# bjack205/rsLQR

Hardware: AMD Instinct MI355X
Metric: LQR solves/sec (nx=12,nu=4,N=256,batch=1024 per GPU) (higher is better)
Workload: dtype f64; 1 GPU; nx=12 nu=4 N=256 batch=1024 per GPU, fp64, factor+solve per step; parallelism=batch-sharded x1, no data-path collective, ranks_seen=1, flags=0, schedule=reduced-fused2

## Files before the change

### include/ndlqr_hip.h

```cpp
#ifndef NDLQR_HIP_H_
#define NDLQR_HIP_H_

#include <stddef.h>
#include <stdint.h>

#ifdef __cplusplus
extern "C" {
#endif

typedef struct NdlqrHipCtx NdlqrHipCtx;

int ndlqr_hip_device_count(void);
const char* ndlqr_hip_last_error(void);

NdlqrHipCtx* ndlqr_hip_create(int nstates, int ninputs, int nhorizon, int batch, int device);
#define NDLQR_CREATE_NO_PAD 1u
NdlqrHipCtx* ndlqr_hip_create_ex(int nstates, int ninputs, int nhorizon, int batch, int device, unsigned create_flags);
void ndlqr_hip_destroy(NdlqrHipCtx* ctx);
int ndlqr_hip_set_flags(NdlqrHipCtx* ctx, unsigned flags);
unsigned ndlqr_hip_get_flags(const NdlqrHipCtx* ctx);
int ndlqr_hip_set_stream(NdlqrHipCtx* ctx, void* hip_stream);
void* ndlqr_hip_get_stream(NdlqrHipCtx* ctx);

int ndlqr_hip_upload_inputs(NdlqrHipCtx* ctx, int p0, int count, const double* AB,
// ... 90 lines not shown
int ndlqr_hip_download_selection(NdlqrHipCtx* ctx, int knot0, int nknots, unsigned blocks, double* out);
int ndlqr_hip_time_shard_top_doubles(NdlqrHipCtx* ctx, int G);
int ndlqr_hip_time_shard_factor(NdlqrHipCtx* ctx, int g, int G);
int ndlqr_hip_time_shard_export(NdlqrHipCtx* ctx, int G, double* buf);
int ndlqr_hip_time_shard_import(NdlqrHipCtx* ctx, int G, const double* buf);
int ndlqr_hip_time_shard_finish(NdlqrHipCtx* ctx, int g, int G);
void* ndlqr_hip_host_alloc(size_t bytes);
void ndlqr_hip_host_free(void* p);
void* ndlqr_hip_device_alloc(size_t bytes);
void ndlqr_hip_device_free(void* p);
int ndlqr_hip_copy(void* dst, const void* src, size_t bytes);

int ndlqr_hip_download_solutions(NdlqrHipCtx* ctx, int p0, int count, double* soln);
int ndlqr_hip_download_rhs_blocks(NdlqrHipCtx* ctx, int p, double* z_full);
int ndlqr_hip_download_factors(NdlqrHipCtx* ctx, int p, double* fact);
int ndlqr_hip_factors_valid(const NdlqrHipCtx* ctx);
int ndlqr_hip_pack_solutions_device(NdlqrHipCtx* ctx, double* dst);
int ndlqr_hip_kkt_residual(NdlqrHipCtx* ctx, double* res, double* bnorm);
int ndlqr_hip_cholesky_failures(NdlqrHipCtx* ctx);
int ndlqr_hip_download_failure_counts(NdlqrHipCtx* ctx, int* counts);
const char* ndlqr_hip_schedule(const NdlqrHipCtx* ctx);
int ndlqr_hip_compact_level1(const NdlqrHipCtx* ctx);
int ndlqr_hip_level1_paired(const NdlqrHipCtx* ctx);

int ndlqr_hip_profile_slots(NdlqrHipCtx* ctx);
int ndlqr_hip_profile_get(NdlqrHipCtx* ctx, int slot, char* name, int name_cap, double* total_ms,
                          int* launches);
int ndlqr_hip_profile_reset(NdlqrHipCtx* ctx);

int ndlqr_hip_gemm(int tA, int tB, int m, int n, int k, double alpha, const double* A, int lda,
                   const double* B, int ldb, double beta, double* C, int ldc);
int ndlqr_hip_potrf_lower(int n, double* A, int lda);
int ndlqr_hip_potrs_lower(int n, int nrhs, const double* L, int ldl, double* B, int ldb);
int ndlqr_hip_trsv_lower(int n, int nrhs, const double* L, int ldl, double* B, int ldb, int transposed);

#ifdef __cplusplus
}
#endif
#endif
```

### rslqr_amd/api.py

```python
import ctypes as C
import os
import re

import numpy as np

from . import build as _build

FLAG_STRICT_FP = 1
FLAG_GENERIC = 2
FLAG_PROFILE = 4
FLAG_KEEP_FACT = 8
FLAG_KEEP_RECORDS = 16
SOLN_LAMBDA, SOLN_STATE, SOLN_INPUT, SOLN_ONLY = 1, 2, 4, 8
GRAD_A, GRAD_B, GRAD_Q, GRAD_R, GRAD_q, GRAD_r, GRAD_d, GRAD_x0 = 1, 2, 4, 8, 16, 32, 64, 128
GRAD_NAMES = ("A", "B", "Q", "R", "q", "r", "d", "x0")
GRADD_A, GRADD_B, GRADD_Q, GRADD_H, GRADD_R, GRADD_q, GRADD_r, GRADD_d, GRADD_x0 = 1, 2, 4, 8, 16, 32, 64, 128, 256
GRAD_DENSE_NAMES = ("A", "B", "Q", "H", "R", "q", "r", "d", "x0")

ERR_INVALID = -1
ERR_NO_DEVICE = -2
ERR_NOT_SPD = -3

dp = C.POINTER(C.c_double)

# ... 285 lines not shown
    proto("ndlqr_BatchSetBoxAcceleration", ci, vp, ci, cd, cd)
    proto("ndlqr_CopyBatchBoxAcceleration", ci, vp, C.POINTER(ci), C.POINTER(ci), dp, C.POINTER(ci))
    proto("ndlqr_SolveBatchBoxAdjoint", ci, vp, dp, C.POINTER(NdLqrBoxSettingsFull), C.POINTER(ci), C.POINTER(ci))
    proto("ndlqr_BatchBoundGradients", ci, vp, C.c_uint, dp, dp, dp, dp)
    proto("ndlqr_PolishBatchBoxConstrained", ci, vp, C.POINTER(NdLqrPolishSettings), C.POINTER(ci), C.POINTER(ci))
    proto("ndlqr_hip_download_polish_codes", ci, vp, C.POINTER(C.c_ubyte))
    proto("ndlqr_SolveBatchPolishedAdjoint", ci, vp, dp, C.POINTER(NdLqrPolishSettings), C.POINTER(ci), C.POINTER(ci))
    proto("ndlqr_hip_factor_count", C.c_ulonglong, vp)
    proto("ndlqr_hip_set_stream", ci, vp, vp)
    proto("ndlqr_hip_get_stream", vp, vp)
    proto("ndlqr_hip_profile_slots", ci, vp)
    proto("ndlqr_hip_profile_get", ci, vp, ci, C.c_char_p, ci, dp, C.POINTER(ci))
    proto("ndlqr_hip_profile_reset", ci, vp)
    proto("ndlqr_hip_device_pointers", ci, vp, C.POINTER(vp))
    proto("ndlqr_hip_staged_io", ci, vp, C.POINTER(dp), C.POINTER(dp), C.POINTER(dp), C.POINTER(dp))
    proto("ndlqr_hip_download_rhs_blocks", ci, vp, ci, dp)
    proto("ndlqr_hip_upload_inputs", ci, vp, ci, ci, dp, dp, dp)
    proto("ndlqr_hip_factors_valid", ci, vp)
    proto("ndlqr_hip_schedule", C.c_char_p, vp)
    if hasattr(L, "ndlqr_hip_compact_level1"):
        proto("ndlqr_hip_compact_level1", C.c_int, vp)
    if hasattr(L, "ndlqr_hip_level1_paired"):
        proto("ndlqr_hip_level1_paired", C.c_int, vp)
    proto("ndlqr_hip_set_pipeline_depth", ci, vp, ci)
    proto("ndlqr_hip_pipeline_depth", ci, vp)
    proto("ndlqr_hip_pack_solutions_device", ci, vp, vp)
    proto("ndlqr_hip_gemm", ci, ci, ci, ci, ci, ci, cd, dp, ci, dp, ci, cd, dp, ci)
    proto("ndlqr_hip_potrf_lower", ci, ci, dp, ci)
    proto("ndlqr_hip_potrs_lower", ci, ci, ci, dp, ci, dp, ci)
    proto("ndlqr_hip_trsv_lower", ci, ci, ci, dp, ci, dp, ci, ci)
    _LIB = L
    return L


def pinned_empty(shape):
    import weakref
    count = int(np.prod(shape))
    L = lib()
    ptr = L.ndlqr_HostAlloc(max(count, 1) * 8)
    if not ptr:
        raise MemoryError("ndlqr_HostAlloc(%d bytes) failed" % (count * 8))
    buf = (C.c_double * max(count, 1)).from_address(ptr)
    arr = np.ctypeslib.as_array(buf)[:count].reshape(shape)
    weakref.finalize(buf, L.ndlqr_HostFree, C.c_void_p(ptr))
    return arr

# ... 788 lines not shown
        err = self.L.ndlqr_CopyBatchCholeskyFailureCounts(self.h, out.ctypes.data_as(C.POINTER(C.c_int)))
        if err:
            raise RuntimeError("ndlqr_CopyBatchCholeskyFailureCounts failed: %d" % err)
        return out

    def profile(self):
        out = {}
        for slot in range(self.L.ndlqr_hip_profile_slots(self.ctx)):
            name = C.create_string_buffer(64)
            ms, cnt = C.c_double(0), C.c_int(0)
            self.L.ndlqr_hip_profile_get(self.ctx, slot, name, 64, C.byref(ms), C.byref(cnt))
            out[name.value.decode()] = (ms.value, cnt.value)
        return out

    def schedule(self):
        return self.L.ndlqr_hip_schedule(self.ctx).decode()

    def compact_level1(self):
        return hasattr(self.L, "ndlqr_hip_compact_level1") and bool(self.L.ndlqr_hip_compact_level1(self.ctx))

    def level1_paired(self):
        return hasattr(self.L, "ndlqr_hip_level1_paired") and bool(self.L.ndlqr_hip_level1_paired(self.ctx))

    def set_pipeline_depth(self, depth):
        return self.L.ndlqr_hip_set_pipeline_depth(self.ctx, depth)

    def pipeline_depth(self):
        return self.L.ndlqr_hip_pipeline_depth(self.ctx)

    def profile_reset(self):
        self.L.ndlqr_hip_profile_reset(self.ctx)
```

### rslqr_amd/csrc/hip_context.hpp

```cpp
#pragma once
#include <hip/hip_runtime.h>

#include <cstdio>
#include <cstdlib>
#include <cstring>
#include <initializer_list>
#include <string>
#include <utility>
#include <vector>

#include "ndlqr.h"
#include "ndlqr_hip.h"

#include "kernels_common.hpp"

#pragma GCC visibility push(hidden)
int ndlqr_hip_fail(const char* what, hipError_t e);
struct NdlqrHipCtx;
int ndlqr_hip_ensure_F(NdlqrHipCtx* c);
#pragma GCC visibility pop
#define HIP_TRY(expr)                                                  \
  do {                                                                 \
    hipError_t e_ = (expr);                                            \
    if (e_ != hipSuccess) return ndlqr_hip_fail(#expr, e_);            \
// ... 6 lines not shown
  if (lds <= kLdsDefaultDynamic) return hipSuccess;
  return hipFuncSetAttribute(reinterpret_cast<const void*>(kernel), hipFuncAttributeMaxDynamicSharedMemorySize, (int)lds);
}


enum { SLOT_LEAF = 0, SLOT_SEP, SLOT_SCHUR, SLOT_BOUNDARY, SLOT_APPLY, SLOT_BOTTOM, SLOT_UPPER, SLOT_TOP, SLOT_COUNT };

struct PendingEvent {
  int slot;
  hipEvent_t start, stop;
};

enum class Family { None, Small, GenericReduced, GenericKnot };

struct KeptState {
  Family family = Family::None;
  bool time_shard = false;
  bool rec_complete = false;
  bool rec_compact = false;
  bool fact_valid = false;
  const char* schedule = "none";
  bool rec1_compact = false;
  bool level1_paired = false;
  void forget_factorisation() { rec_complete = fact_valid = false; }
};

struct CapturedChain {
  hipGraphExec_t exec = nullptr;
  unsigned flags = 0;
  hipStream_t stream = nullptr;
  unsigned apply = 0;
  void reset() {
    if (exec) (void)hipGraphExecDestroy(exec);
    exec = nullptr;
  }
};

struct KnotSlice {
  int knot0 = 0, nknots = 0;
  unsigned blocks = 7u;
  bool valid(int N, unsigned allowed) const {
    return knot0 >= 0 && nknots > 0 && knot0 + nknots <= N && (blocks & 7u) && !(blocks & ~allowed);
  }
  size_t width(const ndlqr::Dims& u) const {
    return ((blocks & 1u) ? u.n : 0) + ((blocks & 2u) ? u.n : 0) + ((blocks & 4u) ? u.m : 0);
  }
// ... 58 lines not shown
  DevBuf<double> red;
  DevBuf<double> ytop;
  DevBuf<double> z;
  DevBuf<double> rhs;
  DevBuf<double> xfer;
  DevBuf<int> tree_cnt;
  PinnedBuf<int> h_fail;
  hipStream_t stream = nullptr;
  hipEvent_t ev_start = nullptr, ev_stop = nullptr;
  unsigned long long rhs_gen[4] = {};
  CapturedChain graph;
  bool ready = false;
  hipError_t ensure_xfer(const ndlqr::Dims& u) { return xfer.ensure((size_t)u.batch * u.N * u.rows + (size_t)u.batch * u.n); }
};


struct DevKnobs {
  int rowbcast = -1;
  int tree = -1;
  int backsub_cols = -1;
  int fuse2 = -1;
  int compact1 = -1;
  int pair1 = -1;
  int pipeline = 2;
  bool no_top = false;
  int top_levels = 3;
  bool no_mfma = false;
  int sep_threads = 0;
  int mult_threads = 0;
  bool no_reduced_generic = false;
  bool no_pad = false;
  bool alt_priority_set = false;
  int alt_priority = 0;
};

struct AdjointState {
  DevBuf<double> rhs, z;
  DevBuf<double> save;
  unsigned long long gen = 0;
  unsigned long long rhs_stamp = 0;
  hipError_t ensure_save(const ndlqr::Dims& d) { return save.ensure(2 * (size_t)d.batch * d.N * d.n); }
  hipError_t ensure(const ndlqr::Dims& d, hipStream_t st) {
    return first_error({rhs.ensure(doubles_z(d)), z.ensure_zeroed(doubles_z(d), st), ensure_save(d)});
  }
};

// ... 308 lines not shown
```

### rslqr_amd/csrc/kernels_bottom_reduced.hpp

```cpp
#pragma once
#include "kernels_dpp.hpp"
#include "kernels_small.hpp"

namespace ndlqr {

typedef double acc4_t __attribute__((ext_vector_type(4)));

template <int NX>
struct McPitch {
  static constexpr int SP = 18, WP = 17;
};

template <int NX, class Hook>
__device__ __forceinline__ void factor_tail_mc(const int lane, const acc4_t& c, const double (&ra)[(NX + 3) / 4],
                                               const double (&rb)[(NX + 3) / 4], const double* Wm, acc4_t& X0,
                                               acc4_t& X1, Hook hook) {
  constexpr int KS = (NX + 3) / 4, WP = McPitch<NX>::WP;
  int lane_o = lane;
  asm volatile("" : "+v"(lane_o));
  const int li = lane_o & 15, lk = lane_o >> 4;
  double wt[KS], wa[KS], b0[KS];
#pragma unroll
  for (int q = 0; q < KS; ++q) {
    wt[q] = Wm[(4 * q + lk) * WP + li];
// ... 439 lines not shown
template <int NX>
__device__ __forceinline__ double* lstore_of(const int store_l, double* F, double* rec, const Dims& d, const int b,
                                             const int level, const int s) {
  return store_l == 2 ? rb_lrec<NX>(rec, d, b, s) : (store_l ? Fblk(F, d, b, level, s + 1) : nullptr);
}

template <int NX, int NU, bool BOTTOM = true>
struct alignas(16) ReducedLds {
  static constexpr int W = NX + NU, ROWS = 2 * NX + NU, WP = (W % 2 == 0) ? W + 2 : W;
  static constexpr int SLOT = RedSlot<NX>::SIZE, NSC = McWyLayout<NX>::SIZE;
  static constexpr int NB0 = BOTTOM ? 4 * NX * WP : 0, NB1 = SLOT + NX * WP;
  static constexpr int NB2 = BOTTOM ? McPairLayout<NX>::SIZE : 0;
  static constexpr int NB3 = BOTTOM ? McPairYLayout<NX>::SIZE : 0;
  static constexpr int NB01 = (NB0 > NB1 ? NB0 : NB1) > NSC ? (NB0 > NB1 ? NB0 : NB1) : NSC;
  static constexpr int NB23 = NB2 > NB3 ? NB2 : NB3;
  static constexpr int NBUF = NB01 > NB23 ? NB01 : NB23;
  static constexpr int NRQ = BOTTOM ? 4 * W : (W + NX + 1) / 2 * 2, NRH = BOTTOM ? 4 * ROWS : (NX + W + 2 * NX + 1) / 2 * 2;
  double buf[NBUF];
  double rq[NRQ];
  double rh[NRH];
#ifdef NDLQR_DEV_LDS_PAD
  double dev_pad[BOTTOM ? NDLQR_DEV_LDS_PAD / 8 : 1];
#endif
};

template <int NX, int NU, bool TREE, class LdsT, bool EXT = false>
__device__ __forceinline__ void reduced_separator_mc(const Dims& d, const int l, const int base, const int b,
                                                     const int lane, const double* __restrict__ AB,
                                                     const double* __restrict__ QR,
                                                     const double* __restrict__ rhs, double* red,
                                                     double* __restrict__ rec, double* F, int* __restrict__ info,
                                                     const int store_l, LdsT& lds, const double* slot_ext = nullptr) {
  constexpr int W = NX + NU, NN = NX * NX, KSN = (NX + 3) / 4;
  constexpr int WP = ReducedLds<NX, NU>::WP, SLOT = RedSlot<NX>::SIZE;
  const double* slot = EXT ? slot_ext : lds.buf;
  double* abs_ = lds.buf + SLOT;
  double* rq = lds.rq;
  double* zs = lds.rh;
  static_assert(LdsT::NRQ >= W + NX && LdsT::NRH >= NX + W + 2 * NX, "the shared arrays are large enough for a level");
  const int N = d.N;
  const int T = 2 << l, s = base + (1 << l) - 1;
  const bool hasA = base > 0, hasB = base + T < N;
  const int li = lane & 15, lk = lane >> 4;
  const int ri = li < NX ? li : NX - 1;
  SEG_INIT();
  const bool leftchild = (base & T) == 0;
// ... 173 lines not shown
  using PY = McPairYLayout<NX>;
  constexpr int KSN = (NX + 3) / 4;
  int lane = lane_in;
  asm volatile("" : "+v"(lane));
  const int li = lane & 15, lk = lane >> 4;
  const bool hasA = k0 > 0, hasB = k0 + 4 < d.N, leftchild = (k0 & 4) == 0;
  RedSlot<NX> sa = red_slot<NX>(red, d, b, hasA ? k0 - 1 : 3);
  RedSlot<NX> sb = red_slot<NX>(red, d, b, hasB ? k0 + 3 : 3);
  if (slotA) sa.p = slotA;
  if (slotB) sb.p = slotB;
  double y0[KSN], y1[KSN];
  acc4_t Z0 = {0.0, 0.0, 0.0, 0.0}, Z1 = {0.0, 0.0, 0.0, 0.0};
#pragma unroll
  for (int q = 0; q < KSN; ++q) {
    y0[q] = buf[PY::tile(0, 0) + (4 * q + lk) * PY::YP + li];
    y1[q] = buf[PY::tile(0, 1) + (4 * q + lk) * PY::YP + li];
    Z0[q] = y0[q]; Z1[q] = y1[q];
  }
  acc4_t g00, g01, g11, unused;
  gram_mc<NX, true, true, false, true>(y0, y1, Z0, Z1, g00, g01, unused, g11);
  push_mc<NX>(lane, hasA, hasB, leftchild, sa, sb, g00, g01, g11, hd.park_a, hd.cb_t, hd.park_b11, StorePlain(), StorePlain());
}

template <int NX, int NU, bool TREE, bool REDIRECT, bool C1 = false, bool P1 = false>
__device__ __forceinline__ void bottom_group_mc(const Dims& d, const int k0, const int b, const int lane,
                                                const double* __restrict__ AB, const double* __restrict__ QR,
                                                const double* __restrict__ rhs, double* red, double* __restrict__ rec,
                                                double* F, int* __restrict__ info, const int store_l, const int compact0,
                                                ReducedLds<NX, NU>& lds, double* slotA, double* slotB,
                                                const bool with_m = false, acc4_t* c_m = nullptr,
                                                Pair1Hand* hand = nullptr);
template <int NX, int NU, bool C1 = false, bool P1 = false>
__global__ __launch_bounds__(128) __attribute__((amdgpu_waves_per_eu(4))) void bottom8_reduced_mc(
    Dims d, const double* __restrict__ AB, const double* __restrict__ QR, const double* __restrict__ rhs, double* red,
    double* __restrict__ rec, int* __restrict__ info) {
  __shared__ ReducedLds<NX, NU> lds[2];
  __shared__ __attribute__((aligned(16))) double mslot[RedSlot<NX>::SIZE];
  const int wave = __builtin_amdgcn_readfirstlane(threadIdx.x >> 6), b = blockIdx.y;
  const int kw = (blockIdx.x + d.xoff) * 8;
  int lane = threadIdx.x & 63;
  for (int e = threadIdx.x; e < RedSlot<NX>::SIZE; e += 128) mslot[e] = 0.0;
  __syncthreads();
  acc4_t c_m = {0.0, 0.0, 0.0, 0.0};
  if constexpr (P1) {
    static_assert(C1, "the paired pass is the Y-only pass of compact level-1 records");
    static_assert(McPair1Layout<NX>::SIZE <= ReducedLds<NX, NU>::NBUF, "tile and couplings of t fit the wavefront's buffer");
    Pair1Hand hd;
    bottom_group_mc<NX, NU, false, true, true, true>(d, kw + 4 * wave, b, lane, AB, QR, rhs, red, rec, nullptr, info, 0, 1,
                                                     lds[wave], nullptr, nullptr, wave == 0, &c_m, &hd);
    pair1_exchange_mc<NX>(lane, hd.c_t, hd.ca_t, hd.cb_t, lds[wave].buf);
    __syncthreads();
    if (wave == 0) {
      double* rec_t0 = rec + ((size_t)b * d.N + kw + 1) * (2 * NX * NX + NX);
      if (chol_pair1_y_mc<NX>(lane, lds[0].buf, lds[1].buf, rec_t0, rec_t0 + 4 * (2 * NX * NX + NX)) &&
          (lane == 0 || lane == 32))
        flag_failure(info, d, b);
    }
    __syncthreads();
    pair1_tail_mc<NX, NU>(d, kw + 4 * wave, b, lane, red, lds[wave].buf, hd, wave == 1 ? mslot : nullptr,
                          wave == 0 ? mslot : nullptr);
  } else {
  bottom_group_mc<NX, NU, false, true, C1>(d, kw + 4 * wave, b, lane, AB, QR, rhs, red, rec, nullptr, info, 0, 1, lds[wave],
                                       wave == 1 ? mslot : nullptr, wave == 0 ? mslot : nullptr, wave == 0, &c_m);
  }
  asm volatile("s_waitcnt vmcnt(0)" ::: "memory");
  __syncthreads();
  asm volatile("" : "+v"(lane));
  if (wave == 0) reduced_eliminate_pass_mc<NX, NU>(d, kw, b, lane, c_m, mslot, info, lds[0].buf);
  __syncthreads();
  reduced_eliminate_tail_mc<NX, NU>(d, kw, b, lane, wave == 0, red, rec, lds[0].buf);
}

template <int NX>
__device__ __forceinline__ void backsub_top_body(const Dims& d, const int b, const int t,
                                                 const double* __restrict__ recs, double* __restrict__ ytop,
                                                 double* ytop_lds, const int bp = -1, const double* zsep = nullptr);
template <int NX, int NU>
__global__ __launch_bounds__(256) __attribute__((amdgpu_waves_per_eu(4))) void reduced_top_mc(Dims d, const int l0, const double* __restrict__ AB,
                                                      const double* __restrict__ QR, const double* __restrict__ rhs,
                                                      double* red, double* __restrict__ rec, double* F,
                                                      int* __restrict__ info, const int store_l,
                                                      double* __restrict__ ytop) {
  __shared__ ReducedLds<NX, NU, false> lds[4];
  const int wave = __builtin_amdgcn_readfirstlane(threadIdx.x >> 6), b = blockIdx.x;
  for (int l = l0, s0 = 0; l < d.K;) {
    int lane = threadIdx.x & 63;
    asm volatile("" : "+v"(lane));
    const int cnt = d.N >> (l + 1);
    if (wave + s0 < cnt)
      reduced_separator_mc<NX, NU, true>(d, l, (wave + s0) * (2 << l), b, lane, AB, QR, rhs, red, rec, F, info, store_l,
                                         lds[wave]);
    s0 += 4;
    if (s0 < cnt) continue;
    s0 = 0;
    ++l;
    asm volatile("s_waitcnt vmcnt(0)" ::: "memory");
    __syncthreads();
  }
  if (ytop) backsub_top_body<NX>(d, b, threadIdx.x, rec, ytop, reinterpret_cast<double*>(&lds[0]), -1, nullptr);
}

template <int NX, int NU, bool TREE, bool REDIRECT, bool C1, bool P1>
__device__ __forceinline__ void bottom_group_mc(const Dims& d, const int k0, const int b, const int lane,
                                                const double* __restrict__ AB, const double* __restrict__ QR,
                                                const double* __restrict__ rhs, double* red, double* __restrict__ rec,
                                                double* F, int* __restrict__ info, const int store_l, const int compact0,
                                                ReducedLds<NX, NU>& lds, double* slotA, double* slotB,
                                                const bool with_m, acc4_t* c_m, Pair1Hand* hand) {
  static_assert(!P1 || (C1 && REDIRECT && !TREE), "the paired level-1 pass: the fused bottom launch with compact level-1 records");
  constexpr int W = NX + NU, ROWS = 2 * NX + NU, NN = NX * NX, KSN = (NX + 3) / 4;
  constexpr int REC = 2 * NN + NX;
  constexpr int WP = ReducedLds<NX, NU>::WP;
  double* abs_ = lds.buf;
  double* rq = lds.rq;
  double* rh = lds.rh;
  const int N = d.N;
  const int li = lane & 15, lk = lane >> 4;
  const int ri = li < NX ? li : NX - 1;
  const bool hasA = k0 > 0, hasB = k0 + 4 < N;
  SEG_INIT();

  {
    const double* abm = AB + ((size_t)b * N + k0) * NX * W;
    const double* q0 = QR + ((size_t)b * N + k0) * W;
    const double* r0 = rhs + ((size_t)b * N + k0) * ROWS;
    constexpr int NQ = 4 * W, IQ = (NQ + 63) / 64, NR = 4 * ROWS, IR = (NR + 63) / 64;
    double qv[IQ], rv[IR];
#pragma unroll
    for (int it = 0; it < IQ; ++it) { const int e = lane + 64 * it; qv[it] = q0[e < NQ ? e : NQ - 1]; }
#pragma unroll
    for (int it = 0; it < IR; ++it) { const int e = lane + 64 * it; rv[it] = r0[e < NR ? e : NR - 1]; }
    if constexpr (W % 2 == 0) {
      constexpr int NA = 4 * NX * W / 2, IA = (NA + 63) / 64;
      double2 t[IA];
#pragma unroll
      for (int it = 0; it < IA; ++it) {
        const int e = lane + 64 * it;
        t[it] = reinterpret_cast<const double2*>(abm)[e < NA ? e : NA - 1];
      }
#pragma unroll
      for (int it = 0; it < IA; ++it) {
        const int e = lane + 64 * it, ec = e < NA ? e : NA - 1, row = ec / (W / 2), c2 = ec - row * (W / 2);
        reinterpret_cast<double2*>(&abs_[row * WP])[c2] = t[it];
      }
    } else {
      constexpr int NA = 4 * NX * W, IA = (NA + 63) / 64;
      double t[IA];
#pragma unroll
      for (int it = 0; it < IA; ++it) { const int e = lane + 64 * it; t[it] = abm[e < NA ? e : NA - 1]; }
#pragma unroll
      for (int it = 0; it < IA; ++it) { const int e = lane + 64 * it; abs_[e < NA ? e : NA - 1] = t[it]; }
    }
#pragma unroll
    for (int it = 0; it < IQ; ++it) {
      const int e = lane + 64 * it, ec = e < NQ ? e : NQ - 1, kn = ec / W, c = ec - kn * W;
      rq[ec] = 1.0 / qv[it];
      if (e < NQ && !positive_finite(qv[it]) && !(k0 + kn == N - 1 && c >= NX)) flag_failure(info, d, b);
    }
#pragma unroll
    for (int it = 0; it < IR; ++it) { const int e = lane + 64 * it; rh[e < NR ? e : NR - 1] = rv[it]; }
  }
  wave_lds_sync();
  SEG(20);

  auto none = [](int) { return 0.0; };
  acc4_t c_s0;
// ... 90 lines not shown
  }
  wave_lds_sync();
  SEG(21);

  using Pair = McPairLayout<NX>;
  if (chol_pair_mc<NX>(lane, c_s0, c_s2, lds.buf, store_l ? Fblk(F, d, b, 0, k0 + 1) : nullptr,
                       store_l ? Fblk(F, d, b, 0, k0 + 3) : nullptr) &&
      (lane == 0 || lane == 32))
    flag_failure(info, d, b);
  SEG(30);
  factor_tail_mc<NX>(lane, c_s0, ra0, rb0, lds.buf + Pair::W_A, X0, X1, hook_s0);
  store_record_mc<NX>(myrec, lane, hasA, true, X0, X1);
  factor_tail_mc<NX>(lane, c_s2, ra2, rb2, lds.buf + Pair::W_B, X0, X1, hook_s2);
  store_record_mc<NX>(myrec + 2 * REC, lane, true, hasB, X0, X1);
  SEG(35);
  }
  if constexpr (P1) {
    hand->c_t = c_t; hand->ca_t = ca_t; hand->cb_t = cb_t; hand->park_a = park_a; hand->park_b11 = park_b11;
    return;
  }
  double wcol[NX];
  {
    constexpr int TP = 17;
    static_assert(2 * 16 * TP <= ReducedLds<NX, NU>::NBUF, "both coupling tiles fit the buffer");
    double* ta = lds.buf;
    double* tb = lds.buf + 16 * TP;
    wave_lds_sync();
#pragma unroll
    for (int g = 0; g < 4; ++g) {
      ta[(lk + 4 * g) * TP + li] = -ca_t[g];
      tb[(lk + 4 * g) * TP + li] = -cb_t[g];
    }
    wave_lds_sync();
    const int h = lane & 31;
    const bool is_a = h < NX, is_b = h > NX && h <= 2 * NX;
    const double* src = is_a ? ta + h : tb + (is_b ? h - NX - 1 : 0);
#pragma unroll
    for (int k = 0; k < NX; ++k) wcol[k] = src[k * TP];
    wave_lds_sync();
  }
  const bool leftchild = (k0 & 4) == 0;
  RedSlot<NX> sa = red_slot<NX>(red, d, b, hasA ? k0 - 1 : 3);
  RedSlot<NX> sb = red_slot<NX>(red, d, b, hasB ? k0 + 3 : 3);
  if constexpr (REDIRECT) {
    if (slotA) sa.p = slotA;
    if (slotB) sb.p = slotB;
  }
// ... 79 lines not shown
```

### rslqr_amd/csrc/launch_small.hpp

```cpp
#pragma once
#include "hip_context.hpp"
#include "kernels_leaf.hpp"
#include "kernels_small.hpp"
#include "kernels_bottom_reduced.hpp"
#include "kernels_rowbcast.hpp"

constexpr int kBottomLevels = 2;

struct SmallPlan {
  bool strict, keep;
  bool lean;
  int store_l;
  bool reduced;
  bool tree;
  bool compact;
  bool rowbcast;
  bool fuse2;
  bool compact1;
  bool pair1;
  int level0;
  int ltop;
  int top_l0;
  bool top_sweeps;
  size_t top_lds;
  const char* schedule;
  bool rec_complete, rec_compact;
  bool needs_F;
};

template <int NX, int NU>
constexpr bool kRbBacksubFits = 8 * (2 * NX + NU) <= 256;

static inline unsigned apply_grid(const NdlqrHipCtx* c, const ndlqr::Dims& d) {
  return (unsigned)(c->apply_nblk > 0 ? c->apply_nblk : d.N / 8);
}
static inline ndlqr::Dims apply_dims(const NdlqrHipCtx* c, const ndlqr::Dims& d) {
  ndlqr::Dims da = d;
  if (c->apply_nblk > 0) da.xoff += c->apply_blk0;
  return da;
}

template <int NX, int NU>
// ... 28 lines not shown
  SmallPlan p = {};
  p.strict = strict;
  p.keep = keep;
  p.lean = !strict && !keep && (d.K + 4) * NX <= 256;
  p.store_l = (c->flags & NDLQR_FLAG_KEEP_RECORDS) ? 1 : 0;
  p.rec_complete = !strict && (keep || (p.lean && p.store_l));
  p.level0 = p.ltop = p.top_l0 = d.K;
  p.schedule = p.lean ? "knot-lean" : (strict ? "knot-strict" : "knot-keep");
  if constexpr (ndlqr::P1OnMatrixCores<NX, NU>::value) {
    if (p.lean && s.red) {
      p.reduced = true;
      p.tree = s.tree_cnt && (c->knobs.tree == 1 || (c->knobs.tree < 0 && (size_t)d.batch * (d.N >> 2) <= 2048));
      p.top_lds = sizeof(double) * (size_t)(d.N >> 3) * NX;
      p.compact = !p.tree && d.N >= 16 && kRbBacksubFits<NX, NU> && p.top_lds * (p.store_l ? 4 : 1) <= kLdsMax;
      if (p.compact && p.store_l) p.store_l = 2;
      p.rec_compact = p.compact && p.store_l == 2;
      p.rowbcast = p.compact && !p.store_l && NX <= 16 && NX + NU <= 16 && (c->knobs.rowbcast == 1 || (c->knobs.rowbcast < 0 && NX <= 8));
      p.fuse2 = !p.rowbcast && p.compact && !p.store_l && (c->knobs.fuse2 > 0 || (c->knobs.fuse2 < 0 && NX == 12 && NU == 4));
      p.compact1 = kCompact1Fits<NX, NU> && p.compact && !p.store_l && !p.rowbcast && c->knobs.backsub_cols != 0 &&
                   (c->knobs.compact1 > 0 ||
                    (c->knobs.compact1 < 0 && ((NX == 12 && NU == 4 && p.fuse2) || (NX == 10 && NU == 4))));
      p.pair1 = kPair1Fits<NX, NU> && p.fuse2 && p.compact1 &&
                (c->knobs.pair1 > 0 || (c->knobs.pair1 < 0 && NX == 12 && NU == 4));
      p.schedule = p.tree ? "reduced-tree"
                   : !p.compact ? "reduced-records"
                   : p.store_l ? "reduced-compact-records" : (p.fuse2 ? "reduced-fused2" : "reduced");
      if (!p.tree) {
        const int top_levels = d.K - c->knobs.top_levels >= 3 ? c->knobs.top_levels : 3;
        p.level0 = p.fuse2 ? 3 : 2;
        p.ltop = (d.K >= 5 && !c->knobs.no_top) ? d.K - top_levels : d.K;
        p.top_l0 = (p.fuse2 && p.ltop < 3) ? 3 : p.ltop;
        p.top_sweeps = p.ltop < d.K && p.compact && p.top_lds <= 4 * sizeof(ndlqr::ReducedLds<NX, NU, false>);
      }
    }
  }
  p.needs_F = !(p.reduced && p.store_l != 1);
  return p;
}

template <int NX, int NU, bool STRICT, bool KEEP>
static int launch_small(NdlqrHipCtx* c, const SmallPlan& plan) {
  const ndlqr::Dims& d = c->d;
  BufferSet& s = c->set[c->cur];
  using Sh = ndlqr::SchurShape<NX, NU>;
  constexpr int JB = kBottomLevels;
  const bool lean = plan.lean;
  const int store_l = plan.store_l;
  if constexpr (!STRICT && !KEEP && ndlqr::P1OnMatrixCores<NX, NU>::value) {
    if (plan.reduced) {
      {
        ScopedSlot t(c, SLOT_BOTTOM);
        if (plan.rowbcast) {
          if constexpr (NX <= 16 && NX + NU <= 16)
            hipLaunchKernelGGL((ndlqr::rb_bottom<NX, NU>), dim3(d.N >> 4, d.batch), dim3(64), 0, s.stream, d, c->AB,
                               c->QR, s.rhs, s.red, s.rec, c->info);
        } else if (plan.fuse2) {
          bool done = false;
          if constexpr (kPair1Fits<NX, NU>) {
            if (plan.pair1) {
              hipLaunchKernelGGL((ndlqr::bottom8_reduced_mc<NX, NU, true, true>), dim3(d.N >> 3, d.batch), dim3(128), 0, s.stream,
                                 d, c->AB, c->QR, s.rhs, s.red, s.rec, c->info);
              done = true;
            }
          }
          if constexpr (kCompact1Fits<NX, NU>) {
            if (!done && plan.compact1) {
              hipLaunchKernelGGL((ndlqr::bottom8_reduced_mc<NX, NU, true>), dim3(d.N >> 3, d.batch), dim3(128), 0, s.stream, d,
                                 c->AB, c->QR, s.rhs, s.red, s.rec, c->info);
              done = true;
            }
          }
          if (!done)
            hipLaunchKernelGGL((ndlqr::bottom8_reduced_mc<NX, NU>), dim3(d.N >> 3, d.batch), dim3(128), 0, s.stream, d,
                               c->AB, c->QR, s.rhs, s.red, s.rec, c->info);
        } else if (plan.tree)
          hipLaunchKernelGGL((ndlqr::bottom_reduced_mc<NX, NU, true>), dim3(d.N >> 2, d.batch), dim3(64), 0, s.stream,
                             d, c->AB, c->QR, s.rhs, s.red, s.rec, c->F, c->info, store_l, s.tree_cnt, 0);
        else if (plan.compact) {
          bool done = false;
          if constexpr (kCompact1Fits<NX, NU>) {
            if (plan.compact1) {
              hipLaunchKernelGGL((ndlqr::bottom_reduced_mc<NX, NU, false, true, true>), dim3(d.N >> 2, d.batch), dim3(64), 0,
// ... 208 lines not shown
```

### rslqr_amd/csrc/ndlqr_hip.hip

```cpp
#include "hip_host.hpp"
#include "kernels_generic.hpp"
#include "kernels_mfma.hpp"
#include "launch_reduced.hpp"
#include "kernels_reduced_solve.hpp"
#include "launch_small.hpp"


static thread_local std::string g_last_error = "";

const char* ndlqr_hip_last_error(void) { return g_last_error.c_str(); }

int ndlqr_hip_fail(const char* what, hipError_t e) {
  g_last_error = std::string(what) + ": " + hipGetErrorString(e);
  fprintf(stderr, "ndlqr_hip: %s\n", g_last_error.c_str());
  if (e == hipErrorInvalidConfiguration || e == hipErrorInvalidValue) return NDLQR_ERR_INVALID;
  return NDLQR_ERR_NO_DEVICE;
}
int fail(const char* what, hipError_t e) { return ndlqr_hip_fail(what, e); }
int refuse(const std::string& msg) {
  g_last_error = msg;
  fprintf(stderr, "ndlqr_hip: %s\n", g_last_error.c_str());
  return NDLQR_ERR_INVALID;
}

// ... 53 lines not shown
  }
}

static const SmallInstance* find_small(const ndlqr::Dims& d) {
  for (const SmallInstance* s : kSmallInstances)
    if (s->nx == d.n && s->nu == d.m) return s;
  return nullptr;
}

static size_t bytes_z(const ndlqr::Dims& d) { return sizeof(double) * doubles_z(d); }
static size_t bytes_F(const ndlqr::Dims& d) { return sizeof(double) * doubles_F(d); }

static DevKnobs read_knobs() {
  DevKnobs k;
  const auto num = [](const char* name, int* v) { if (getenv(name)) *v = atoi(getenv(name)); };
  const auto onoff = [](const char* name, int* v) { if (getenv(name)) *v = atoi(getenv(name)) != 0 ? 1 : 0; };
  num("NDLQR_PIPELINE", &k.pipeline);
  onoff("NDLQR_TREE", &k.tree);
  onoff("NDLQR_ROWBCAST", &k.rowbcast);
  onoff("NDLQR_FUSE2", &k.fuse2);
  onoff("NDLQR_BACKSUB_COLS", &k.backsub_cols);
  onoff("NDLQR_COMPACT1", &k.compact1);
  onoff("NDLQR_PAIR1", &k.pair1);
  k.no_mfma = getenv("NDLQR_NO_MFMA") != nullptr;
  k.no_top = getenv("NDLQR_NO_TOP") != nullptr;
  num("NDLQR_TOP_LEVELS", &k.top_levels);
  if (k.top_levels < 3 || k.top_levels > 5) k.top_levels = 3;
  num("NDLQR_SEP_THREADS", &k.sep_threads);
  num("NDLQR_MULT_THREADS", &k.mult_threads);
  k.no_reduced_generic = getenv("NDLQR_DEV_NO_REDUCED_GENERIC") != nullptr;
  k.no_pad = getenv("NDLQR_NO_PAD") != nullptr;
  k.alt_priority_set = getenv("NDLQR_ALT_PRIORITY") != nullptr;
  num("NDLQR_ALT_PRIORITY", &k.alt_priority);
  return k;
}

static bool alloc_set(NdlqrHipCtx* c, BufferSet& s, bool slots) {
  const ndlqr::Dims& d = c->d;
  hipError_t e = first_error({hipEventCreate(&s.ev_start), hipEventCreate(&s.ev_stop), s.rec.ensure((size_t)d.batch * d.N * (2 * d.n * d.n + d.n)),
                              s.rhs.ensure(doubles_z(d)), s.h_fail.ensure_zeroed(1)});
  if (e == hipSuccess && slots) {
    const size_t slot_doubles = ((size_t)d.n * (d.n + 1) + 2 * (size_t)d.n * d.n + 2 * d.n + 15) / 16 * 16;
    e = first_error({s.red.ensure_zeroed((size_t)d.batch * (d.N / 4) * slot_doubles, s.stream),
                     s.ytop.ensure((size_t)d.batch * (d.N / 8) * d.n),
                     s.tree_cnt.ensure_zeroed((size_t)d.batch * (d.N / 4), s.stream)});
  }
// ... 562 lines not shown
  if (!inst || d.N < inst->kpb || d.K < 3) return nullptr;
  return inst;
}

static const SmallInstance* kept_instance(const NdlqrHipCtx* c) {
  return c->kept.family == Family::Small ? find_small(c->d) : nullptr;
}

static SolvePlan plan_solve(const NdlqrHipCtx* c) {
  const ndlqr::Dims& d = c->d;
  SolvePlan p = {};
  p.strict = (c->flags & NDLQR_FLAG_STRICT_FP) != 0;
  p.keep = (c->flags & NDLQR_FLAG_KEEP_FACT) != 0;
  p.inst = pick_small(c);
  if (p.inst) {
    p.family = Family::Small;
    p.small = p.inst->plan(c, p.strict, p.keep);
    p.needs_F = p.small.needs_F;
    p.kept.schedule = p.small.schedule;
    p.kept.rec_complete = p.small.rec_complete;
    p.kept.rec_compact = p.small.rec_compact;
    p.kept.rec1_compact = p.small.compact1;
    p.kept.level1_paired = p.small.pair1;
  } else if ((p.red = plan_reduced_generic(c)).ok) {
    p.family = Family::GenericReduced;
    p.needs_red_generic = true;
    p.kept.schedule = p.red.keep ? "generic-reduced-records" : "generic-reduced";
    p.kept.rec_complete = p.red.keep;
  } else {
    p.family = Family::GenericKnot;
    p.rec_as_factors = (c->flags & NDLQR_FLAG_KEEP_RECORDS) && !p.strict;
    p.lean = !p.strict && !p.keep && !p.rec_as_factors;
    p.needs_F = true;
    p.sep = plan_generic_sep(c, p.strict);
    if (p.sep.scratch)
      p.sep_scratch_bytes = sizeof(double) * ((size_t)d.n * (d.n + 1) + (size_t)d.n * (2 * d.n + 1)) * (size_t)d.batch *
                            (d.N / 2 > 0 ? d.N / 2 : 1);
    p.kept.schedule = p.lean ? "generic-lean" : (p.strict ? "generic-strict" : "generic-keep");
  }
  p.kept.family = p.family;
  p.kept.fact_valid = p.keep || p.rec_as_factors || ((c->flags & NDLQR_FLAG_GENERIC) && p.strict);
  p.may_pipeline = !p.needs_F && !(c->flags & (NDLQR_FLAG_PROFILE | NDLQR_FLAG_KEEP_RECORDS | NDLQR_FLAG_KEEP_FACT));
  return p;
}

static int enqueue_solve(NdlqrHipCtx* c, const SolvePlan& plan) {
// ... 793 lines not shown
  for (size_t i = 0; i <= nchunks && e == hipSuccess; ++i) {
    if (i < nchunks) {
      const size_t off = i * chunk, len = total - off < chunk ? total - off : chunk;
      e = hipMemcpyAsync(c->h_stage[i & 1], s.xfer + off, sizeof(double) * len, hipMemcpyDeviceToHost, st);
      if (e == hipSuccess) e = hipEventRecord(done[i & 1], st);
    }
    if (i > 0 && e == hipSuccess) {
      const size_t off = (i - 1) * chunk, len = total - off < chunk ? total - off : chunk;
      e = hipEventSynchronize(done[(i - 1) & 1]);
      if (e == hipSuccess) memcpy(soln + off, c->h_stage[(i - 1) & 1], sizeof(double) * len);
    }
  }
  c->event_pool.push_back(done[0]);
  c->event_pool.push_back(done[1]);
  if (e != hipSuccess) return fail("ndlqr_hip_download_solutions", e);
  return NDLQR_OK;
}

const char* ndlqr_hip_schedule(const NdlqrHipCtx* c) { return c ? c->kept.schedule : "none"; }

int ndlqr_hip_compact_level1(const NdlqrHipCtx* c) { return c && c->kept.rec1_compact ? 1 : 0; }

int ndlqr_hip_level1_paired(const NdlqrHipCtx* c) { return c && c->kept.level1_paired ? 1 : 0; }

int ndlqr_hip_factors_valid(const NdlqrHipCtx* c) { return c && c->kept.fact_valid ? 1 : 0; }

int ndlqr_hip_pack_solutions_device(NdlqrHipCtx* c, double* dst) {
  if (!c || !dst) return NDLQR_ERR_INVALID;
  if (c->z_partial || c->z_invalid) return need_full_solution(c, "ndlqr_hip_pack_solutions_device");
  const ndlqr::Dims& d = c->d;
  HIP_TRY(hipSetDevice(c->device));
  HIP_TRY(launch_pack(c->du, d, KnotSlice(), c->set[c->latest].z, dst, c->set[c->latest].stream, d.batch));
  if (c->cost.dense && !c->cost.mapped(c->soln_gen)) HIP_TRY(cost_map_back(c, dst, 0, d.batch, c->set[c->latest].stream));
  return NDLQR_OK;
}

int ndlqr_hip_kkt_residual(NdlqrHipCtx* c, double* res, double* bnorm) {
  if (!c || !res) return NDLQR_ERR_INVALID;
  if (const int cerr = need_diagonal_cost(c, "ndlqr_hip_kkt_residual")) return cerr;
  if (c->z_partial || c->z_invalid) return need_full_solution(c, "ndlqr_hip_kkt_residual");
  const ndlqr::Dims& d = c->d;
  BufferSet& s = c->set[c->cur];
  HIP_TRY(hipSetDevice(c->device));
  HIP_TRY(c->kkt_out.ensure(2 * (size_t)d.batch));
  double* out = c->kkt_out;
  HIP_TRY(sync_all(c));
// ... 89 lines not shown
```

Measured before the change: 2.028 million solves/s.

## Shrink fused bottom kernel LDS to 16 KB by aliasing level-2 slot and parked tiles

Adds a compact shared-memory layout for the paired level-1 fused bottom kernel. The separate mslot array is aliased into the tail of the wavefront buffers, and the second wave's gram tiles are parked in LDS so that wave 0 can finish the level-2 push. The goal is to fit ten workgroups per CU, raising occupancy (waves_per_eu 5). The cost is extra LDS round trips, odd-stride scalar stores when the padding is odd, and more serialization on wave 0. It is enabled by default whenever pair1 applies.

```diff
diff --git a/include/ndlqr_hip.h b/include/ndlqr_hip.h
--- a/include/ndlqr_hip.h
+++ b/include/ndlqr_hip.h
@@ -136,6 +136,7 @@
 const char* ndlqr_hip_schedule(const NdlqrHipCtx* ctx);
 int ndlqr_hip_compact_level1(const NdlqrHipCtx* ctx);
 int ndlqr_hip_level1_paired(const NdlqrHipCtx* ctx);
+int ndlqr_hip_bottom_lds16(const NdlqrHipCtx* ctx);
 
 int ndlqr_hip_profile_slots(NdlqrHipCtx* ctx);
 int ndlqr_hip_profile_get(NdlqrHipCtx* ctx, int slot, char* name, int name_cap, double* total_ms,
diff --git a/rslqr_amd/api.py b/rslqr_amd/api.py
--- a/rslqr_amd/api.py
+++ b/rslqr_amd/api.py
@@ -331,6 +331,8 @@
         proto("ndlqr_hip_compact_level1", C.c_int, vp)
     if hasattr(L, "ndlqr_hip_level1_paired"):
         proto("ndlqr_hip_level1_paired", C.c_int, vp)
+    if hasattr(L, "ndlqr_hip_bottom_lds16"):
+        proto("ndlqr_hip_bottom_lds16", C.c_int, vp)
     proto("ndlqr_hip_set_pipeline_depth", ci, vp, ci)
     proto("ndlqr_hip_pipeline_depth", ci, vp)
     proto("ndlqr_hip_pack_solutions_device", ci, vp, vp)
@@ -1165,6 +1167,9 @@
     def level1_paired(self):
         return hasattr(self.L, "ndlqr_hip_level1_paired") and bool(self.L.ndlqr_hip_level1_paired(self.ctx))
 
+    def bottom_lds16(self):
+        return hasattr(self.L, "ndlqr_hip_bottom_lds16") and bool(self.L.ndlqr_hip_bottom_lds16(self.ctx))
+
     def set_pipeline_depth(self, depth):
         return self.L.ndlqr_hip_set_pipeline_depth(self.ctx, depth)
 
diff --git a/rslqr_amd/csrc/hip_context.hpp b/rslqr_amd/csrc/hip_context.hpp
--- a/rslqr_amd/csrc/hip_context.hpp
+++ b/rslqr_amd/csrc/hip_context.hpp
@@ -52,6 +52,7 @@
   const char* schedule = "none";
   bool rec1_compact = false;
   bool level1_paired = false;
+  bool bottom_lds16 = false;
   void forget_factorisation() { rec_complete = fact_valid = false; }
 };
 
@@ -156,6 +157,7 @@
   int fuse2 = -1;
   int compact1 = -1;
   int pair1 = -1;
+  int bottom_lds16 = -1;
   int pipeline = 2;
   bool no_top = false;
   int top_levels = 3;
diff --git a/rslqr_amd/csrc/kernels_bottom_reduced.hpp b/rslqr_amd/csrc/kernels_bottom_reduced.hpp
--- a/rslqr_amd/csrc/kernels_bottom_reduced.hpp
+++ b/rslqr_amd/csrc/kernels_bottom_reduced.hpp
@@ -485,6 +485,22 @@
 #ifdef NDLQR_DEV_LDS_PAD
   double dev_pad[BOTTOM ? NDLQR_DEV_LDS_PAD / 8 : 1];
 #endif
+};
+
+template <int NX, int NU>
+struct alignas(16) Bottom8Lds16 {
+  static constexpr int W = NX + NU, ROWS = 2 * NX + NU;
+  static constexpr int NTILE = McPair1Layout<NX>::SIZE > McPairYLayout<NX>::SIZE
+                                   ? (McPair1Layout<NX>::SIZE > McWyLayout<NX>::SIZE ? McPair1Layout<NX>::SIZE : McWyLayout<NX>::SIZE)
+                                   : (McPairYLayout<NX>::SIZE > McWyLayout<NX>::SIZE ? McPairYLayout<NX>::SIZE : McWyLayout<NX>::SIZE);
+  static constexpr int WP = (W % 2 == 0) ? (4 * NX * (W + 2) <= NTILE ? W + 2 : W + 1) : W;
+  static constexpr int NBUF = 4 * NX * WP > NTILE ? 4 * NX * WP : NTILE;
+  static constexpr int NRQ = 4 * W, NRH = 4 * ROWS;
+  static constexpr int MSLOT = 2 * McPairYLayout<NX>::TILE;
+  static_assert(MSLOT % 2 == 0 && MSLOT + RedSlot<NX>::SIZE <= NBUF + NRQ + NRH, "the level-2 slot fits behind the Y tiles");
+  double buf[NBUF];
+  double rq[NRQ];
+  double rh[NRH];
 };
 
 template <int NX, int NU, bool TREE, class LdsT, bool EXT = false>
@@ -704,18 +720,27 @@
   push_mc<NX>(lane, hasA, hasB, leftchild, sa, sb, g00, g01, g11, hd.park_a, hd.cb_t, hd.park_b11, StorePlain(), StorePlain());
 }
 
-template <int NX, int NU, bool TREE, bool REDIRECT, bool C1 = false, bool P1 = false>
+template <int NX, int NU, bool TREE, bool REDIRECT, bool C1 = false, bool P1 = false, class LdsT>
 __device__ __forceinline__ void bottom_group_mc(const Dims& d, const int k0, const int b, const int lane,
                                                 const double* __restrict__ AB, const double* __restrict__ QR,
                                                 const double* __restrict__ rhs, double* red, double* __restrict__ rec,
                                                 double* F, int* __restrict__ info, const int store_l, const int compact0,
-                                                ReducedLds<NX, NU>& lds, double* slotA, double* slotB,
+                                                LdsT& lds, double* slotA, double* slotB,
                                                 const bool with_m = false, acc4_t* c_m = nullptr,
                                                 Pair1Hand* hand = nullptr);
-template <int NX, int NU, bool C1 = false, bool P1 = false>
-__global__ __launch_bounds__(128) __attribute__((amdgpu_waves_per_eu(4))) void bottom8_reduced_mc(
+template <int NX, int NU>
+__device__ __forceinline__ void bottom8_lds16_mc(const Dims& d, const double* __restrict__ AB, const double* __restrict__ QR,
+                                                 const double* __restrict__ rhs, double* red, double* __restrict__ rec,
+                                                 int* __restrict__ info);
+template <int NX, int NU, bool C1 = false, bool P1 = false, bool L16 = false>
+__global__ __launch_bounds__(128) __attribute__((amdgpu_waves_per_eu(L16 ? 5 : 4))) void bottom8_reduced_mc(
     Dims d, const double* __restrict__ AB, const double* __restrict__ QR, const double* __restrict__ rhs, double* red,
     double* __restrict__ rec, int* __restrict__ info) {
+  if constexpr (L16) {
+    static_assert(P1, "the 16 KB layout is that of the paired pass");
+    bottom8_lds16_mc<NX, NU>(d, AB, QR, rhs, red, rec, info);
+    return;
+  }
   __shared__ ReducedLds<NX, NU> lds[2];
   __shared__ __attribute__((aligned(16))) double mslot[RedSlot<NX>::SIZE];
   const int wave = __builtin_amdgcn_readfirstlane(threadIdx.x >> 6), b = blockIdx.y;
@@ -751,6 +776,130 @@
   if (wave == 0) reduced_eliminate_pass_mc<NX, NU>(d, kw, b, lane, c_m, mslot, info, lds[0].buf);
   __syncthreads();
   reduced_eliminate_tail_mc<NX, NU>(d, kw, b, lane, wave == 0, red, rec, lds[0].buf);
+}
+
+struct McParkLayout {
+  static constexpr int A = 0, B = 256, GL = 512, SIZE = 528;
+};
+template <int NX, int NU>
+__device__ __forceinline__ void pair1_tail_park_mc(const Dims& d, const int k0, const int b, const int lane_in,
+                                                   const double* buf, const Pair1Hand& hd, const bool left, double* mslot,
+                                                   double* park) {
+  using PY = McPairYLayout<NX>;
+  using PK = McParkLayout;
+  constexpr int KSN = (NX + 3) / 4;
+  int lane = lane_in;
+  asm volatile("" : "+v"(lane));
+  const int li = lane & 15, lk = lane >> 4;
+  const bool hasA = k0 > 0, hasB = k0 + 4 < d.N;
+  const RedSlot<NX> sm = {mslot};
+  double y0[KSN], y1[KSN];
+  acc4_t Z0 = {0.0, 0.0, 0.0, 0.0}, Z1 = {0.0, 0.0, 0.0, 0.0};
+#pragma unroll
+  for (int q = 0; q < KSN; ++q) {
+    y0[q] = buf[PY::tile(0, 0) + (4 * q + lk) * PY::YP + li];
+    y1[q] = buf[PY::tile(0, 1) + (4 * q + lk) * PY::YP + li];
+    Z0[q] = y0[q]; Z1[q] = y1[q];
+  }
+  acc4_t g00, g01, g11, unused;
+  gram_mc<NX, true, true, false, true>(y0, y1, Z0, Z1, g00, g01, unused, g11);
+  if (left) {
+#pragma unroll
+    for (int g = 0; g < 4; ++g) park[PK::A + 64 * g + lane] = g00[g] + hd.park_a[g];
+    if (li < NX) {
+#pragma unroll
+      for (int g = 0; g < 4; ++g) {
+        const int r = lk + 4 * g;
+        if (!rows_none<NX>(g) && (rows_all<NX>(g) || r < NX)) {
+          if (li <= r) sm.DL()[r * (r + 1) / 2 + li] = g11[g] + hd.park_b11[g];
+          sm.CA()[li * NX + r] = hasA ? g01[g] : 0.0;
+        }
+      }
+      if (lk == NX % 4) sm.gL()[li] = g01[NX / 4] + hd.cb_t[NX / 4];
+    }
+  } else {
+    if (li <= NX) {
+#pragma unroll
+      for (int g = 0; g < 4; ++g) {
+        const int r = lk + 4 * g;
+        if (!rows_none<NX>(g) && (rows_all<NX>(g) || r < NX) && (li <= r || li == NX))
+          (li < NX ? sm.DR() + r * (r + 1) / 2 + li : sm.gR() + r)[0] = g00[g] + hd.park_a[g];
+      }
+    }
+#pragma unroll
+    for (int g = 0; g < 4; ++g) park[PK::B + 64 * g + lane] = g11[g] + hd.park_b11[g];
+    if (li < NX) {
+      if (lk == NX % 4) park[PK::GL + li] = g01[NX / 4] + hd.cb_t[NX / 4];
+#pragma unroll
+      for (int g = 0; g < 4; ++g) {
+        const int r = lk + 4 * g;
+        if (!rows_none<NX>(g) && (rows_all<NX>(g) || r < NX)) sm.CB()[r * NX + li] = hasB ? g01[g] : 0.0;
+      }
+    }
+  }
+}
+template <int NX, int NU>
+__device__ __forceinline__ void reduced_eliminate_gram_park_mc(const Dims& d, const int base, const int b, const int lane,
+                                                               double* red, const double* buf, const double* park) {
+  using P = McWyLayout<NX>;
+  using PK = McParkLayout;
+  constexpr int KS = P::KS;
+  const int N = d.N, T = 8, s = base + 3;
+  const bool hasA = base > 0, hasB = base + T < N, leftchild = (base & T) == 0;
+  const int li = lane & 15, lk = lane >> 4;
+  double y0[KS], y1[KS];
+  acc4_t Z0 = {0.0, 0.0, 0.0, 0.0}, Z1 = {0.0, 0.0, 0.0, 0.0};
+#pragma unroll
+  for (int q = 0; q < KS; ++q) {
+    y0[q] = buf[P::Y0 + (4 * q + lk) * P::YP + li];
+    y1[q] = buf[P::Y1 + (4 * q + lk) * P::YP + li];
+    Z0[q] = y0[q]; Z1[q] = y1[q];
+  }
+  acc4_t pa, pb11, pb01 = {0.0, 0.0, 0.0, 0.0};
+#pragma unroll
+  for (int g = 0; g < 4; ++g) { pa[g] = park[PK::A + 64 * g + lane]; pb11[g] = park[PK::B + 64 * g + lane]; }
+  pb01[NX / 4] = park[PK::GL + li];
+  const RedSlot<NX> sa = red_slot<NX>(red, d, b, hasA ? base - 1 : s);
+  const RedSlot<NX> sb = red_slot<NX>(red, d, b, hasB ? base + T - 1 : s);
+  acc4_t g00, g01, g11, unused;
+  gram_mc<NX, true, true, false, true>(y0, y1, Z0, Z1, g00, g01, unused, g11);
+  push_mc<NX>(lane, hasA, hasB, leftchild, sa, sb, g00, g01, g11, pa, pb01, pb11, StorePlain(), StorePlain());
+}
+
+template <int NX, int NU>
+__device__ __forceinline__ void bottom8_lds16_mc(const Dims& d, const double* __restrict__ AB, const double* __restrict__ QR,
+                                                 const double* __restrict__ rhs, double* red, double* __restrict__ rec,
+                                                 int* __restrict__ info) {
+  using L = Bottom8Lds16<NX, NU>;
+  __shared__ L lds[2];
+  static_assert(sizeof(L) * 2 <= 16384, "ten workgroups per CU");
+  static_assert(McPair1Layout<NX>::SIZE <= L::NBUF, "tile and couplings of t fit the wavefront's buffer");
+  static_assert(L::MSLOT + McParkLayout::SIZE <= L::NBUF + L::NRQ + L::NRH, "the parked tiles fit behind the Y tiles");
+  double* mslot = reinterpret_cast<double*>(&lds[0]) + L::MSLOT;
+  double* park = reinterpret_cast<double*>(&lds[1]) + L::MSLOT;
+  const int wave = __builtin_amdgcn_readfirstlane(threadIdx.x >> 6), b = blockIdx.y;
+  const int kw = (blockIdx.x + d.xoff) * 8;
+  int lane = threadIdx.x & 63;
+  acc4_t c_m = {0.0, 0.0, 0.0, 0.0};
+  Pair1Hand hd;
+  bottom_group_mc<NX, NU, false, true, true, true>(d, kw + 4 * wave, b, lane, AB, QR, rhs, red, rec, nullptr, info, 0, 1,
+                                                   lds[wave], nullptr, nullptr, wave == 0, &c_m, &hd);
+  pair1_exchange_mc<NX>(lane, hd.c_t, hd.ca_t, hd.cb_t, lds[wave].buf);
+  __syncthreads();
+  if (wave == 0) {
+    double* rec_t0 = rec + ((size_t)b * d.N + kw + 1) * (2 * NX * NX + NX);
+    if (chol_pair1_y_mc<NX>(lane, lds[0].buf, lds[1].buf, rec_t0, rec_t0 + 4 * (2 * NX * NX + NX)) &&
+        (lane == 0 || lane == 32))
+      flag_failure(info, d, b);
+  }
+  __syncthreads();
+  pair1_tail_park_mc<NX, NU>(d, kw + 4 * wave, b, lane, lds[wave].buf, hd, wave == 0, mslot, park);
+  __syncthreads();
+  asm volatile("" : "+v"(lane));
+  if (wave == 0) reduced_eliminate_pass_mc<NX, NU>(d, kw, b, lane, c_m, mslot, info, lds[0].buf);
+  __syncthreads();
+  if (wave == 0) reduced_eliminate_gram_park_mc<NX, NU>(d, kw, b, lane, red, lds[0].buf, park);
+  else reduced_eliminate_tail_mc<NX, NU>(d, kw, b, lane, false, red, rec, lds[0].buf);
 }
 
 template <int NX>
@@ -782,17 +931,17 @@
   if (ytop) backsub_top_body<NX>(d, b, threadIdx.x, rec, ytop, reinterpret_cast<double*>(&lds[0]), -1, nullptr);
 }
 
-template <int NX, int NU, bool TREE, bool REDIRECT, bool C1, bool P1>
+template <int NX, int NU, bool TREE, bool REDIRECT, bool C1, bool P1, class LdsT>
 __device__ __forceinline__ void bottom_group_mc(const Dims& d, const int k0, const int b, const int lane,
                                                 const double* __restrict__ AB, const double* __restrict__ QR,
                                                 const double* __restrict__ rhs, double* red, double* __restrict__ rec,
                                                 double* F, int* __restrict__ info, const int store_l, const int compact0,
-                                                ReducedLds<NX, NU>& lds, double* slotA, double* slotB,
+                                                LdsT& lds, double* slotA, double* slotB,
                                                 const bool with_m, acc4_t* c_m, Pair1Hand* hand) {
   static_assert(!P1 || (C1 && REDIRECT && !TREE), "the paired level-1 pass: the fused bottom launch with compact level-1 records");
   constexpr int W = NX + NU, ROWS = 2 * NX + NU, NN = NX * NX, KSN = (NX + 3) / 4;
   constexpr int REC = 2 * NN + NX;
-  constexpr int WP = ReducedLds<NX, NU>::WP;
+  constexpr int WP = LdsT::WP;
   double* abs_ = lds.buf;
   double* rq = lds.rq;
   double* rh = lds.rh;
@@ -823,7 +972,12 @@
 #pragma unroll
       for (int it = 0; it < IA; ++it) {
         const int e = lane + 64 * it, ec = e < NA ? e : NA - 1, row = ec / (W / 2), c2 = ec - row * (W / 2);
-        reinterpret_cast<double2*>(&abs_[row * WP])[c2] = t[it];
+        if constexpr (WP % 2 == 0) {
+          reinterpret_cast<double2*>(&abs_[row * WP])[c2] = t[it];
+        } else {
+          abs_[row * WP + 2 * c2] = t[it].x;
+          abs_[row * WP + 2 * c2 + 1] = t[it].y;
+        }
       }
     } else {
       constexpr int NA = 4 * NX * W, IA = (NA + 63) / 64;
@@ -960,7 +1114,7 @@
   double wcol[NX];
   {
     constexpr int TP = 17;
-    static_assert(2 * 16 * TP <= ReducedLds<NX, NU>::NBUF, "both coupling tiles fit the buffer");
+    static_assert(2 * 16 * TP <= LdsT::NBUF, "both coupling tiles fit the buffer");
     double* ta = lds.buf;
     double* tb = lds.buf + 16 * TP;
     wave_lds_sync();
diff --git a/rslqr_amd/csrc/launch_small.hpp b/rslqr_amd/csrc/launch_small.hpp
--- a/rslqr_amd/csrc/launch_small.hpp
+++ b/rslqr_amd/csrc/launch_small.hpp
@@ -18,6 +18,7 @@
   bool fuse2;
   bool compact1;
   bool pair1;
+  bool lds16;
   int level0;
   int ltop;
   int top_l0;
@@ -92,6 +93,7 @@
                     (c->knobs.compact1 < 0 && ((NX == 12 && NU == 4 && p.fuse2) || (NX == 10 && NU == 4))));
       p.pair1 = kPair1Fits<NX, NU> && p.fuse2 && p.compact1 &&
                 (c->knobs.pair1 > 0 || (c->knobs.pair1 < 0 && NX == 12 && NU == 4));
+      p.lds16 = p.pair1 && c->knobs.bottom_lds16 != 0;
       p.schedule = p.tree ? "reduced-tree"
                    : !p.compact ? "reduced-records"
                    : p.store_l ? "reduced-compact-records" : (p.fuse2 ? "reduced-fused2" : "reduced");
@@ -127,7 +129,11 @@
         } else if (plan.fuse2) {
           bool done = false;
           if constexpr (kPair1Fits<NX, NU>) {
-            if (plan.pair1) {
+            if (plan.lds16) {
+              hipLaunchKernelGGL((ndlqr::bottom8_reduced_mc<NX, NU, true, true, true>), dim3(d.N >> 3, d.batch), dim3(128), 0,
+                                 s.stream, d, c->AB, c->QR, s.rhs, s.red, s.rec, c->info);
+              done = true;
+            } else if (plan.pair1) {
               hipLaunchKernelGGL((ndlqr::bottom8_reduced_mc<NX, NU, true, true>), dim3(d.N >> 3, d.batch), dim3(128), 0, s.stream,
                                  d, c->AB, c->QR, s.rhs, s.red, s.rec, c->info);
               done = true;
diff --git a/rslqr_amd/csrc/ndlqr_hip.hip b/rslqr_amd/csrc/ndlqr_hip.hip
--- a/rslqr_amd/csrc/ndlqr_hip.hip
+++ b/rslqr_amd/csrc/ndlqr_hip.hip
@@ -99,6 +99,7 @@
   onoff("NDLQR_BACKSUB_COLS", &k.backsub_cols);
   onoff("NDLQR_COMPACT1", &k.compact1);
   onoff("NDLQR_PAIR1", &k.pair1);
+  onoff("NDLQR_BOTTOM_LDS16", &k.bottom_lds16);
   k.no_mfma = getenv("NDLQR_NO_MFMA") != nullptr;
   k.no_top = getenv("NDLQR_NO_TOP") != nullptr;
   num("NDLQR_TOP_LEVELS", &k.top_levels);
@@ -707,6 +708,7 @@
     p.kept.rec_compact = p.small.rec_compact;
     p.kept.rec1_compact = p.small.compact1;
     p.kept.level1_paired = p.small.pair1;
+    p.kept.bottom_lds16 = p.small.lds16;
   } else if ((p.red = plan_reduced_generic(c)).ok) {
     p.family = Family::GenericReduced;
     p.needs_red_generic = true;
@@ -1546,6 +1548,7 @@
 int ndlqr_hip_compact_level1(const NdlqrHipCtx* c) { return c && c->kept.rec1_compact ? 1 : 0; }
 
 int ndlqr_hip_level1_paired(const NdlqrHipCtx* c) { return c && c->kept.level1_paired ? 1 : 0; }
+int ndlqr_hip_bottom_lds16(const NdlqrHipCtx* c) { return c && c->kept.bottom_lds16 ? 1 : 0; }
 
 int ndlqr_hip_factors_valid(const NdlqrHipCtx* c) { return c && c->kept.fact_valid ? 1 : 0; }
 
```

After: 2.125 million solves/s (median of 6 runs). 1.05x the previous value.
